# ShinobuAmasaki/forgex

Hardware: NVIDIA B200
Metric: input_GBps (higher is better)
Workload: dtype u8

## Files before the change

### forgex_b200/csrc/fx_cabi.cu

```cuda
#include <cuda_runtime.h>

#include <algorithm>
#include <atomic>
#include <cstdio>
#include <cstdlib>
#include <cstring>
#include <mutex>
#include <new>
#include <string>
#include <vector>

#include "../../include/forgex_b200.h"
#include "fx_internal.hpp"
#include "fx_kernels.cuh"

using namespace fxk;

namespace {

std::atomic<long long> g_launches{0};

constexpr int STATE_CAP = 16383;
constexpr int SPARSE_STATE_CAP = 2048;
constexpr int DIRECT_LIMIT_BYTES = 40 * 1024;
// ... 413 lines not shown
    if (n == 0) return FX_OK;
    if (p->prog.nfa_engine) return launch_nfa_bool(p, OP, buf, nullptr, stride, n, out, s);
    Plan pl;
    int rc = make_plan(p, pl);
    if (rc) return rc;
    int generic = gated_mode(p, OP);
    p->last_sparse = 0;
    p->last_compact = 0;
    if (OP == 1 && !generic && p->sparse && stride > 0 && n < (1ll << 31) && env_int("FX_SPARSE", 1)) {
        p->last_sparse = 1;
        return launch_sparse(p, pl, buf, nullptr, n, n * stride, out, s, stride);
    }
    if (pl.kind == 3 && p->compact && !generic && pl.kp.prefix_mode == 0 && stride >= 16 && stride % 16 == 0 &&
        reinterpret_cast<uintptr_t>(buf) % 16 == 0 && env_int("FX_COMPACT", 1)) {
        const bool in_smem = p->residency != FX_TABLE_GLOBAL;
        const size_t smem = 256 + (in_smem ? (size_t)p->prog.bt.nstates * 8 + 16 : 0);
        auto kern_s = k_bool_fixed_compact<OP, true>;
        auto kern_g = k_bool_fixed_compact<OP, false>;
        int bps = 0;
        int rc2 = in_smem ? occupancy_grid(kern_s, 1024, smem, p->dev.sm_count, bps) : occupancy_grid(kern_g, 1024, smem, p->dev.sm_count, bps);
        if (rc2) return rc2;
        long long want = (n + 1023) / 1024, cap = (long long)p->dev.sm_count * bps * 2;
        const int grid = (int)(want < cap ? want : cap);
        if (in_smem) kern_s<<<grid, 1024, smem, s>>>(pl.kp, p->dev.ctab4, p->dev.cmap4, buf, n, stride, out);
        else kern_g<<<grid, 1024, smem, s>>>(pl.kp, p->dev.ctab4, p->dev.cmap4, buf, n, stride, out);
        g_launches++;
        p->last_compact = in_smem ? 1 : 2;
        p->last_residency = in_smem ? FX_TABLE_SMEM : FX_TABLE_GLOBAL;
        return cuda_status(cudaGetLastError());
    }
    if (pl.kind == 0) return launch_fixed_v<OP, 0>(p, pl, buf, n, stride, out, s, generic);
    if (pl.kind == 2) return launch_fixed_v<OP, 2>(p, pl, buf, n, stride, out, s, generic);
    return launch_fixed_v<OP, 3>(p, pl, buf, n, stride, out, s, generic);
}

struct Tiling {
    int spt, cap;
    int64_t ntiles;
    int table_smem;
    size_t smem;
};

Tiling make_tiling(const Plan& pl, int64_t n, int64_t total, int extra = 0, int64_t max_cap = 1 << 30) {
    Tiling t;
    int64_t avg = n > 0 ? (total + n - 1) / n : 1;
    if (avg < 1) avg = 1;
    t.table_smem = (int)staged_bytes(pl);
    const int64_t per_cta = (227 * 1024) / 4 - 1024;
    int64_t spt = 0, cap = 0;
    for (int iter = 0; iter < 2; iter++) {
        int64_t fixed = tile_offset(t.table_smem, (int)(spt ? spt : 256)) + 64 + 128 + extra;
        cap = per_cta - fixed;
        if (cap < 8192) cap = 8192;
        if (cap > max_cap) cap = max_cap;
        cap &= ~(int64_t)127;
        spt = (cap * 4 / 5) / avg;
        spt = (spt / 32) * 32;
        if (spt < 32) spt = 32;
        if (spt > 2048) spt = 2048;
    }
    t.spt = (int)spt;
    t.cap = (int)cap;
    t.ntiles = (n + spt - 1) / spt;
    t.smem = (size_t)tile_offset(t.table_smem, t.spt) + (size_t)extra + (size_t)t.cap + 64;
    return t;
}

template <int OP, int KIND>
int launch_ragged_t(fx_pattern* p, const Plan& pl, const uint8_t* buf, const int64_t* off, int64_t n, int64_t total,
                    uint8_t* out, cudaStream_t s, int generic) {
    auto kern = k_bool_ragged<OP, KIND>;
    Tiling t = make_tiling(pl, n, total);
    int bps = 0;
    int rc = occupancy_grid(kern, 256, t.smem, p->dev.sm_count, bps);
    if (rc) return rc;
    long long cap = (long long)p->dev.sm_count * bps;
    int grid = (int)(t.ntiles < cap ? t.ntiles : cap);
    if (grid < 1) grid = 1;
    kern<<<grid, 256, t.smem, s>>>(pl.kp, buf, off, n, total, out, t.spt, t.cap, t.ntiles, t.table_smem, generic);
    g_launches++;
    return cuda_status(cudaGetLastError());
}

template <int KIND, int NR, bool HIGH, bool TWO>
int launch_sparse_t(fx_pattern* p, const Plan& pl, const SparseParams& sp, int table_bytes, const uint8_t* buf,
                    const int64_t* off, int64_t n, int64_t total, uint8_t* out, cudaStream_t s, int64_t stride) {
    auto kern = k_in_sparse<KIND, NR, HIGH, TWO>;
    int64_t avg = n > 0 ? (total + n - 1) / n : 1;
    if (avg < 1) avg = 1;
    int64_t want = (24 * 1024) / avg;
    const int spt = (int)(want < 32 ? 32 : want > 4096 ? 4096 : want);
    const int64_t ntiles = (n + spt - 1) / spt;
    const int table_smem = KIND == 3 ? 0 : (table_bytes + 15) & ~15;
    const size_t smem = (size_t)sparse_shared_head(table_smem) + 8 * (size_t)SPARSE_WARP_BYTES;
    int bps = 0;
    int rc = occupancy_grid(kern, 256, smem, p->dev.sm_count, bps);
    if (rc) return rc;
    long long cap = (long long)p->dev.sm_count * bps;
    long long wantg = (ntiles + 7) / 8;
    int grid = (int)(wantg < cap ? wantg : cap);
    if (grid < 1) grid = 1;
    const int prezeroed = sp.start_nul == 0 && pl.kp.q0_accepting == 0;
    if (prezeroed) CUDA_TRY(cudaMemsetAsync(out, 0, (size_t)n, s));
    kern<<<grid, 256, smem, s>>>(pl.kp, sp, buf, off, n, total, out, spt, ntiles, table_smem, prezeroed, stride);
    g_launches++;
    return cuda_status(cudaGetLastError());
}

template <int KIND, bool HIGH>
int launch_sparse_k(fx_pattern* p, const Plan& pl, const SparseParams& sp, int tb, const uint8_t* buf, const int64_t* off,
                    int64_t n, int64_t total, uint8_t* out, cudaStream_t s, int64_t stride) {
    if (p->first.sweep_nr == 1 && p->first.sweep_lo[0] == p->first.sweep_hi[0]) {
        const SparseParams& one = sp;
        if (p->first.two) return launch_sparse_t<KIND, -1, HIGH, true>(p, pl, one, tb, buf, off, n, total, out, s, stride);
        return launch_sparse_t<KIND, -1, HIGH, false>(p, pl, one, tb, buf, off, n, total, out, s, stride);
    }
    switch (p->first.sweep_nr) {
        case 0: return launch_sparse_t<KIND, 0, true, false>(p, pl, sp, tb, buf, off, n, total, out, s, stride);
        case 1: return launch_sparse_t<KIND, 1, HIGH, false>(p, pl, sp, tb, buf, off, n, total, out, s, stride);
        case 2: return launch_sparse_t<KIND, 2, HIGH, false>(p, pl, sp, tb, buf, off, n, total, out, s, stride);
        case 3: return launch_sparse_t<KIND, 3, HIGH, false>(p, pl, sp, tb, buf, off, n, total, out, s, stride);
        default: return launch_sparse_t<KIND, 4, HIGH, false>(p, pl, sp, tb, buf, off, n, total, out, s, stride);
    }
}

void fill_sweep(const FirstSet& f, SparseParams& sp) {
    for (int r = 0; r < 4; r++) {
        const int k = r < f.sweep_nr ? r : 0;
        sp.add_lo[r] = (0x80u - f.sweep_lo[k]) * 0x01010101u;
        sp.add_hi[r] = (0x7Fu - f.sweep_hi[k]) * 0x01010101u;
    }
    if (f.sweep_nr == 1 && f.sweep_lo[0] == f.sweep_hi[0]) sp.add_lo[0] = f.sweep_lo[0] * 0x01010101u;
    sp.second = f.second * 0x01010101u;
    sp.second_high = f.second_high ? 0xFFFFFFFFu : 0u;
}

int launch_sparse(fx_pattern* p, const Plan& pl, const uint8_t* buf, const int64_t* off, int64_t n, int64_t total,
                  uint8_t* out, cudaStream_t s, int64_t stride) {
    const fx::ByteTable& at = p->anchored.bt;
    const DeviceTables& d = p->dev;
    SparseParams sp;
    sp.table = d.a_table; sp.classmap = d.a_classmap; sp.flags = d.a_flags;
    sp.table_words = (int)at.table.size();
    sp.row_shift = at.row_shift;
    sp.q0 = at.q0; sp.start_nul = at.start_nul;
    fill_sweep(p->first, sp);
    const int tb = (int)at.table.size() * 2;
    const bool smem_table = p->residency != FX_TABLE_GLOBAL && tb <= 24 * 1024;
    if (smem_table)
        return p->first.high ? launch_sparse_k<2, true>(p, pl, sp, tb, buf, off, n, total, out, s, stride)
                             : launch_sparse_k<2, false>(p, pl, sp, tb, buf, off, n, total, out, s, stride);
    return p->first.high ? launch_sparse_k<3, true>(p, pl, sp, tb, buf, off, n, total, out, s, stride)
                         : launch_sparse_k<3, false>(p, pl, sp, tb, buf, off, n, total, out, s, stride);
}

template <int OP>
int launch_ragged(fx_pattern* p, const uint8_t* buf, const int64_t* off, int64_t n, int64_t total, uint8_t* out,
                  cudaStream_t s) {
    if (n < 0 || total < 0) return FX_ERR_BAD_ARGUMENT;
    if (n == 0) return FX_OK;
    if (p->prog.nfa_engine) return launch_nfa_bool(p, OP, buf, off, 0, n, out, s);
    Plan pl;
    int rc = make_plan(p, pl);
    if (rc) return rc;
    int generic = gated_mode(p, OP);
    p->last_sparse = 0;
    if (OP == 1 && !generic && p->sparse && n < (1ll << 31) && env_int("FX_SPARSE", 1)) {
        p->last_sparse = 1;
        return launch_sparse(p, pl, buf, off, n, total, out, s, 0);
    }
    if (pl.kind == 0) return launch_ragged_t<OP, 0>(p, pl, buf, off, n, total, out, s, generic);
    if (pl.kind == 2) return launch_ragged_t<OP, 2>(p, pl, buf, off, n, total, out, s, generic);
    return launch_ragged_t<OP, 3>(p, pl, buf, off, n, total, out, s, generic);
}

template <int KIND>
int launch_regex_ragged_t(fx_pattern* p, const Plan& pl, const uint8_t* buf, const int64_t* off, int64_t n,
                          int64_t total, int64_t* from, int64_t* to, cudaStream_t s) {
    auto kern = k_regex_ragged<KIND>;
    Tiling t = make_tiling(pl, n, total);
    int bps = 0;
    int rc = occupancy_grid(kern, 256, t.smem, p->dev.sm_count, bps);
    if (rc) return rc;
    long long cap = (long long)p->dev.sm_count * bps;
    int grid = (int)(t.ntiles < cap ? t.ntiles : cap);
    if (grid < 1) grid = 1;
    kern<<<grid, 256, t.smem, s>>>(pl.kp, buf, off, n, total, from, to, t.spt, t.cap, t.ntiles, t.table_smem);
    g_launches++;
    return cuda_status(cudaGetLastError());
// ... 1055 lines not shown
```

### forgex_b200/csrc/fx_kernels.cuh

```cuda
#pragma once
#include <cuda_runtime.h>
#include <stdint.h>

namespace fxk {

static constexpr uint32_t W_ACC = 0x8000u, W_INTER = 0x4000u, W_STATE = 0x3FFFu;
static constexpr uint32_t SF_ACC = 1, SF_END = 2, SF_INTER = 4, SF_MATCHED = 8, SF_FAILACC1 = 16;

struct KParams {
    const uint16_t* table;
    const uint8_t* classmap;
    const uint8_t* flags;
    const uint8_t* lits;
    int table_words;
    int nstates;
    int row_shift;
    int start, start_nul, q0, q0_accepting;
    int all_len, pre_len, suf_len;
    int all_active;
    int pre_active, suf_active;
    const uint16_t* a_table;
    const uint8_t* a_classmap;
    const uint8_t* a_flags;
    int a_row_shift, a_start_nul, a_q0;
// ... 706 lines not shown
    int64_t t1;
};
__device__ __forceinline__ TileCtx load_tile(const uint8_t* __restrict__ buf,
                                             const int64_t* __restrict__ offsets, int64_t n, int64_t total, int64_t t,
                                             int spt, int cap, uint8_t* tile, int32_t* s_off, uint32_t mbar,
                                             uint32_t& phase) {
    TileCtx c;
    c.first = t * spt;
    c.count = (int)((n - c.first) < spt ? (n - c.first) : spt);
    const int64_t t0 = __ldg(offsets + c.first);
    const int64_t tend = __ldg(offsets + c.first + c.count);
    c.t1 = tend - t0 > cap ? t0 + cap : tend;
    bool armed = false;
    c.base = t0;
    if (t0 < c.t1) c.base = stage_tile(buf, t0, c.t1, total, tile, mbar, armed);
    for (int i = threadIdx.x; i <= c.count; i += blockDim.x) {
        const int64_t o = __ldg(offsets + c.first + i);
        s_off[i] = o > c.t1 ? OFF_BEYOND : (int32_t)(o - c.base);
    }
    if (armed) { mbar_wait(mbar, phase); phase ^= 1; }
    __syncthreads();
    return c;
}

__host__ __device__ __forceinline__ int tile_offset(int table_smem_bytes, int spt) {
    return (16 + 256 + table_smem_bytes + (spt + 4) * 4 + spt + 127) & ~127;
}

template <int OP, int KIND>
__global__ void __launch_bounds__(256, 4) k_bool_ragged(KParams p, const uint8_t* __restrict__ buf,
                                                        const int64_t* __restrict__ offsets, int64_t n, int64_t total,
                                                        uint8_t* __restrict__ out, int spt, int cap, int64_t ntiles,
                                                        int table_smem_bytes, int generic) {
    extern __shared__ __align__(128) uint8_t smem[];
    uint8_t* s_cmap = smem + 16;
    uint8_t* s_table = smem + 16 + 256;
    int32_t* s_off = reinterpret_cast<int32_t*>(smem + 16 + 256 + table_smem_bytes);
    uint8_t* s_res = reinterpret_cast<uint8_t*>(s_off + spt + 4);
    uint8_t* tile = smem + tile_offset(table_smem_bytes, spt);
    const uint32_t mbar = smem_u32(smem);
    Table<KIND> T = stage_table<KIND>(p, s_table, s_cmap);
    if (threadIdx.x == 0) mbar_init(mbar, 1);
    __syncthreads();
    uint32_t phase = 0;
    const uint32_t tile_addr = smem_u32(tile);
    for (int64_t t = blockIdx.x; t < ntiles; t += gridDim.x) {
        const TileCtx c = load_tile(buf, offsets, n, total, t, spt, cap, tile, s_off, mbar, phase);
        for (int i = threadIdx.x; i < c.count; i += blockDim.x) {
            const int32_t r0 = s_off[i], r1 = s_off[i + 1];
            bool r;
            if (generic || r1 == OFF_BEYOND) {
                const int64_t o0 = __ldg(offsets + c.first + i), o1 = __ldg(offsets + c.first + i + 1);
                r = eval_bool_slow<OP>(p, buf + o0, o1 - o0);
            } else {
                const int len = r1 - r0;
                const uint32_t a = tile_addr + (uint32_t)r0;
                if (degenerate_text<OP>(len, len ? lds_u8(a) : 0)) r = p.q0_accepting != 0;
                else {
                    uint32_t high = 0;
                    r = result_flag(p, walk_smem(T, (uint32_t)p.start, a, len, high));
                    if (OP == 1 && r && p.prefix_mode == 1 && (high & 0x80808080u))
                        r = recheck_in_with_prefix(p, buf + (c.base + r0), len);
                }
            }
            s_res[i] = r ? 1 : 0;
        }
        __syncthreads();
        for (int i = threadIdx.x; i < c.count; i += blockDim.x) out[c.first + i] = s_res[i];
        __syncthreads();
    }
}

struct SparseParams {
    const uint16_t* table;
    const uint8_t* classmap;
    const uint8_t* flags;
    int table_words, row_shift, q0, start_nul;
    uint32_t add_lo[4];
    uint32_t add_hi[4];
    uint32_t second;
    uint32_t second_high;
};

static constexpr int SPARSE_WARP_BYTES = 2 * 64 * 16;
static constexpr int SPARSE_PARAM_BYTES = 1024;
__host__ __device__ __forceinline__ int sparse_shared_head(int table_smem_bytes) { return ((256 + table_smem_bytes + 15) & ~15) + SPARSE_PARAM_BYTES; }

template <int NR, bool HIGH>
__device__ __forceinline__ uint32_t first_mask(const SparseParams& sp, uint32_t w) {
    uint32_t m = 0;
    if (NR == -1) {
        const uint32_t x = w ^ sp.add_lo[0];
        m = (x - 0x01010101u) & ~x;
    } else {
        const uint32_t y = w & 0x7F7F7F7Fu;
#pragma unroll
        for (int r = 0; r < NR; r++) m |= (y + sp.add_lo[r]) & ~(y + sp.add_hi[r]);
    }
    if (HIGH) m |= w;
    return m;
}
__device__ __forceinline__ uint32_t lead_sel(const SparseParams& sp) { return sp.second_high ? 0xBA98u : 0x4444u; }
template <bool LEAD>
__device__ __forceinline__ uint32_t second_zero(const SparseParams& sp, uint32_t w, uint32_t sel) {
    uint32_t z = w ^ sp.second;
    if (LEAD) {
        uint32_t s;
        asm("prmt.b32 %0, %1, 0, %2;" : "=r"(s) : "r"(w), "r"(sel));
        z &= ~s;
    }
    return z;
}
__device__ __forceinline__ uint32_t pair_mask(const SparseParams& sp, uint32_t w, uint32_t z, uint32_t z_next) {
    const uint32_t t = (w ^ sp.add_lo[0]) | __funnelshift_r(z, z_next, 8);
    return (t - 0x01010101u) & ~t;
}
template <int NR, bool HIGH, bool TWO>
__device__ __forceinline__ uint32_t unit_any(const SparseParams& sp, const uint4& a, const uint4& b, uint32_t& seen,
                                             uint32_t z_next = 0u) {
    const uint32_t w[8] = {a.x, a.y, a.z, a.w, b.x, b.y, b.z, b.w};
    const uint32_t all = w[0] | w[1] | w[2] | w[3] | w[4] | w[5] | w[6] | w[7];
    seen |= all;
    uint32_t any = 0;
    if (TWO) {
        const uint32_t sel = lead_sel(sp);
#pragma unroll
        for (int k = 7; k >= 0; k--) {
            const uint32_t z = second_zero<!HIGH>(sp, w[k], sel);
            any |= pair_mask(sp, w[k], z, z_next);
            z_next = z;
        }
        if (HIGH) any |= all;
    } else {
#pragma unroll
        for (int k = 0; k < 8; k++) any |= first_mask<NR, false>(sp, w[k]);
        if (HIGH) any |= all;
    }
    return any & 0x80808080u;
}
__device__ __forceinline__ uint32_t pack_byte_flags(uint32_t m) { return ((((m >> 7) & 0x01010101u) * 0x00204081u) >> 21) & 0xFu; }

template <class TBL, class FETCH>
__device__ __forceinline__ bool attempt_wins(const Anchored& A, const TBL& T, FETCH fetch, int64_t len, uint32_t st, int64_t pos) {
    uint32_t w = st;
    int64_t seq = 0;
    bool inter = false;
    for (int64_t j = pos; j <= len; j++) {
        const uint32_t b = j < len ? fetch(j) : 0u;
        if (inter && (b & 0xC0) != 0x80) {
            const uint32_t f = __ldg(A.flags + (w & W_STATE));
            if (f & ((SF_FAILACC1 << (int)(j - seq)) - SF_FAILACC1)) return true;
            inter = false;
        }
        const uint32_t nw = T.next(w & W_STATE, b);
        if ((nw & W_INTER) && !inter) seq = j;
        inter = (nw & W_INTER) != 0;
        w = nw;
        if (w & W_ACC) return true;
        if ((w & W_STATE) == 0) return false;
    }
    return false;
}

struct SparseCtx {
    const uint8_t* buf;
    const int64_t* offsets;
    int64_t stride;
    uint8_t* out;
    int64_t n, total;
    int spt;
    uint4* units;
    uint4* starts;
};
static constexpr uint32_t SPARSE_START = 0, SPARSE_RECHECK = 2;
__device__ __forceinline__ int64_t sparse_off(const int64_t* __restrict__ offsets, int64_t stride, int64_t i) {
    return offsets ? __ldg(offsets + i) : i * stride;
}

template <int KIND>
__device__ __forceinline__ Table<KIND> sparse_table(const SparseParams& sp, uint32_t s_table, uint32_t s_cmap) {
    Table<KIND> T;
    T.s_table = s_table; T.s_cmap = s_cmap; T.g_table = sp.table; T.g_cmap = sp.classmap; T.shift = sp.row_shift;
    return T;
}

template <int KIND>
__device__ __noinline__ void sparse_run_starts(const KParams& p, const SparseParams& sp, uint32_t s_table, uint32_t s_cmap,
                                               const SparseCtx& c, int count) {
    const Table<KIND> T = sparse_table<KIND>(sp, s_table, s_cmap);
    const int lane = threadIdx.x & 31;
    const Anchored A{sp.flags, sp.start_nul, sp.q0};
    __syncwarp();
    if (lane < count) {
        const uint4 e = c.starts[lane];
        const int64_t first = (int64_t)e.x * c.spt;
        const int64_t* off = c.offsets + first;
        const uint32_t kind = e.y & 7u;
        const int64_t val = (int64_t)(((unsigned long long)e.w << 32) | e.z);
        if (c.offsets == nullptr) {
            const int64_t s = kind == SPARSE_START ? val / c.stride : val;
            const uint8_t* str = c.buf + (first + s) * c.stride;
            bool win;
            if (kind == SPARSE_START) {
                win = !(c.stride == 1 && __ldg(str) == 0x20) &&
                      attempt_wins(A, T, FetchGlobal{str}, c.stride, (uint32_t)sp.q0, val - s * c.stride);
                if (win && p.prefix_mode == 1 && (e.y >> 31)) win = recheck_in_with_prefix(p, str, c.stride);
                if (win) c.out[first + s] = 1;
            } else {
                c.out[first + s] = recheck_in_with_prefix(p, str, c.stride) ? 1 : 0;
            }
        } else if (kind == SPARSE_START) {
            const int cnt = (int)((c.n - first) < c.spt ? (c.n - first) : c.spt);
            int64_t vlo = __ldg(off), vhi = __ldg(off + cnt);
            const int64_t gpos = vlo + val;
            int s = 0, sh = cnt;
            for (int iter = 0; sh - s > 1; iter++) {
                int mid = (s + sh) >> 1;
                if (iter < 6) {
                    mid = s + (int)((float)(gpos - vlo) * (float)(sh - s) / (float)(vhi - vlo));
                    mid = mid <= s ? s + 1 : mid >= sh ? sh - 1 : mid;
                }
                const int64_t v = __ldg(off + mid);
                if (v <= gpos) { s = mid; vlo = v; } else { sh = mid; vhi = v; }
            }
            const int64_t o0 = __ldg(off + s), o1 = __ldg(off + s + 1);
            const uint8_t* str = c.buf + o0;
            if (!(o1 - o0 == 1 && __ldg(str) == 0x20)) {
                bool win = attempt_wins(A, T, FetchGlobal{str}, o1 - o0, (uint32_t)sp.q0, gpos - o0);
                if (win && p.prefix_mode == 1 && (e.y >> 31)) win = recheck_in_with_prefix(p, str, o1 - o0);
                if (win) c.out[first + s] = 1;
            }
        } else {
            const int64_t o0 = __ldg(off + val), o1 = __ldg(off + val + 1);
            c.out[first + val] = recheck_in_with_prefix(p, c.buf + o0, o1 - o0) ? 1 : 0;
        }
    }
    __syncwarp();
}

template <int KIND, int NR, bool HIGH, bool TWO>
__device__ __noinline__ int sparse_run_units(const KParams& p, const SparseParams& sp, uint32_t s_table, uint32_t s_cmap,
                                             const SparseCtx& c, int count, int sqn) {
    const Table<KIND> T = sparse_table<KIND>(sp, s_table, s_cmap);
    const int lane = threadIdx.x & 31;
    const uint32_t FULL = 0xffffffffu;
    __syncwarp();
    uint32_t cand = 0, tile = 0, flag = 0;
    int64_t P = 0, t0 = 0;
    if (lane < count) {
        const uint4 e = c.units[lane];
        tile = e.x; flag = e.y & 0x80000000u;
        const int64_t first = (int64_t)e.x * c.spt;
        const int cnt = (int)((c.n - first) < c.spt ? (c.n - first) : c.spt);
        t0 = sparse_off(c.offsets, c.stride, first);
        const int64_t tend = sparse_off(c.offsets, c.stride, first + cnt);
        const uintptr_t gbuf = reinterpret_cast<uintptr_t>(c.buf);
        const uintptr_t ua = ((gbuf + (uintptr_t)t0) & ~(uintptr_t)31) + ((((uintptr_t)e.w << 32) | e.z) << 5);
        const uint4 v0 = __ldg(reinterpret_cast<const uint4*>(ua)), v1 = __ldg(reinterpret_cast<const uint4*>(ua + 16));
        P = (int64_t)ua - (int64_t)gbuf;
        if (TWO) {
            const uint32_t sel = lead_sel(sp);
            uint32_t z_next = P + 32 < tend ? second_zero<true>(sp, __ldg(reinterpret_cast<const uint8_t*>(ua + 32)), sel) : 0u;
            const uint32_t w[8] = {v0.x, v0.y, v0.z, v0.w, v1.x, v1.y, v1.z, v1.w};
#pragma unroll
            for (int k = 7; k >= 0; k--) {
                const uint32_t z = second_zero<true>(sp, w[k], sel);
                cand |= pack_byte_flags(pair_mask(sp, w[k], z, z_next) | (HIGH ? w[k] : 0u)) << (4 * k);
                z_next = z;
            }
        } else {
            cand = pack_byte_flags(first_mask<NR, HIGH>(sp, v0.x)) | (pack_byte_flags(first_mask<NR, HIGH>(sp, v0.y)) << 4) |
                   (pack_byte_flags(first_mask<NR, HIGH>(sp, v0.z)) << 8) | (pack_byte_flags(first_mask<NR, HIGH>(sp, v0.w)) << 12) |
                   (pack_byte_flags(first_mask<NR, HIGH>(sp, v1.x)) << 16) | (pack_byte_flags(first_mask<NR, HIGH>(sp, v1.y)) << 20) |
                   (pack_byte_flags(first_mask<NR, HIGH>(sp, v1.z)) << 24) | (pack_byte_flags(first_mask<NR, HIGH>(sp, v1.w)) << 28);
        }
        if (P < t0) cand &= 0xFFFFFFFFu << (int)(t0 - P);
        if (P + 32 > tend) cand &= (P >= tend) ? 0u : (0xFFFFFFFFu >> (int)(P + 32 - tend));
    }
    while (__any_sync(FULL, cand != 0)) {
        bool sv = false;
        int64_t pos = 0;
        if (cand) {
            pos = P + __ffs(cand) - 1;
            cand &= cand - 1;
            const uint32_t b = __ldg(c.buf + pos);
            const uint32_t w1 = T.next((uint32_t)sp.q0, b);
            if (w1 & (W_ACC | W_INTER)) sv = true;
            else if (w1 & W_STATE) {
                const uint32_t b1 = pos + 1 < c.total ? __ldg(c.buf + pos + 1) : 0u;
                sv = ((T.next(w1, b1) | T.next(w1, 0u)) & (W_STATE | W_ACC)) != 0;
            }
        }
        const uint32_t m = __ballot_sync(FULL, sv);
        if (m) {
            const unsigned long long rel = (unsigned long long)(pos - t0);
            if (sv) c.starts[sqn + __popc(m & ((1u << lane) - 1))] = make_uint4(tile, SPARSE_START | flag, (uint32_t)rel, (uint32_t)(rel >> 32));
            sqn += __popc(m);
            if (sqn >= 32) {
                sparse_run_starts<KIND>(p, sp, s_table, s_cmap, c, 32);
                if (lane < sqn - 32) { const uint4 x = c.starts[32 + lane]; c.starts[lane] = x; }
                sqn -= 32;
                __syncwarp();
            }
        }
    }
    __syncwarp();
    return sqn;
}

static constexpr int SPARSE_CTAS_PER_SM = 4, SPARSE_ROWS = 4;

template <int NR, bool HIGH, bool TWO, bool WHOLE>
__device__ __forceinline__ uint32_t sweep_group(const SparseParams& sp, uintptr_t sbase, int r, int lim, uint32_t& seen) {
    const int lane = threadIdx.x & 31;
    uint4 va[SPARSE_ROWS], vb[SPARSE_ROWS];
#pragma unroll
    for (int k = 0; k < SPARSE_ROWS; k++) {
        const int u = ((r + k) << 5) + lane;
        const uintptr_t a = sbase + ((uintptr_t)(uint32_t)u << 5);
        if (WHOLE || u < lim) {
            va[k] = ldg_nc_v4(reinterpret_cast<const void*>(a));
            vb[k] = ldg_nc_v4(reinterpret_cast<const void*>(a + 16));
        } else {
            va[k] = make_uint4(0, 0, 0, 0); vb[k] = va[k];
        }
    }
    uint32_t zn[SPARSE_ROWS];
    if (TWO) {
        const uint32_t sel = lead_sel(sp);
        uint32_t z0[SPARSE_ROWS];
#pragma unroll
        for (int k = 0; k < SPARSE_ROWS; k++) z0[k] = second_zero<true>(sp, va[k].x, sel);
#pragma unroll
        for (int k = 0; k < SPARSE_ROWS; k++) {
            const uint32_t give = lane != 0 ? z0[k] : k + 1 < SPARSE_ROWS ? z0[k + 1] : 0u;
            zn[k] = __shfl_sync(0xffffffffu, give, (lane + 1) & 31);
            if (!WHOLE && ((r + k) << 5) + lane + 1 >= lim) zn[k] = 0u;
        }
    }
    uint32_t bits = 0;
#pragma unroll
    for (int k = 0; k < SPARSE_ROWS; k++) {
        const int u = ((r + k) << 5) + lane;
        const uint32_t h = (WHOLE || u < lim) ? unit_any<NR, HIGH, TWO>(sp, va[k], vb[k], seen, TWO ? zn[k] : 0u) : 0u;
        bits |= (h ? 1u : 0u) << k;
    }
    return bits;
}

template <int KIND, int NR, bool HIGH, bool TWO>
__global__ void __launch_bounds__(256, SPARSE_CTAS_PER_SM) k_in_sparse(KParams p, SparseParams sp, const uint8_t* __restrict__ buf,
                                                                     const int64_t* __restrict__ offsets, int64_t n, int64_t total,
                                                                     uint8_t* __restrict__ out, int spt, int64_t ntiles,
                                                                     int table_smem_bytes, int prezeroed, int64_t stride) {
    extern __shared__ __align__(128) uint8_t smem[];
    uint8_t* s_cmap = smem;
    uint8_t* s_table = smem + 256;
    const int warp = threadIdx.x >> 5, lane = threadIdx.x & 31;
    uint4* s_units = reinterpret_cast<uint4*>(smem + sparse_shared_head(table_smem_bytes) + warp * SPARSE_WARP_BYTES);
    uint4* s_starts = s_units + 64;
    KParams anch = p;
    anch.table = sp.table; anch.classmap = sp.classmap; anch.table_words = sp.table_words; anch.row_shift = sp.row_shift;
    Table<KIND> T = stage_table<KIND>(anch, s_table, s_cmap);
    static_assert(sizeof(KParams) + sizeof(SparseParams) + 8 * sizeof(SparseCtx) <= SPARSE_PARAM_BYTES, "parameter block");
    uint8_t* s_params = smem + sparse_shared_head(table_smem_bytes) - SPARSE_PARAM_BYTES;
    KParams* sh_p = reinterpret_cast<KParams*>(s_params);
    SparseParams* sh_sp = reinterpret_cast<SparseParams*>(s_params + sizeof(KParams));
    SparseCtx* sh_c = reinterpret_cast<SparseCtx*>(s_params + sizeof(KParams) + sizeof(SparseParams)) + warp;
    if (threadIdx.x == 0) { *sh_p = p; *sh_sp = sp; }
    if (lane == 0) {
        sh_c->buf = buf; sh_c->offsets = offsets; sh_c->stride = stride; sh_c->out = out; sh_c->n = n; sh_c->total = total;
        sh_c->spt = spt;
        sh_c->units = s_units; sh_c->starts = s_starts;
    }
    __syncthreads();
    const Anchored A{sp.flags, sp.start_nul, sp.q0};
    const uint32_t FULL = 0xffffffffu;
    const int nt = (int)ntiles;

    enum { ST_NEW = 0, ST_SWEEP = 1, ST_STRINGS = 2, ST_PUSH = 3 };
    int t = blockIdx.x * 8 + warp;
    int st = ST_NEW, it = 0;
    int uqn = 0, sqn = 0;
    int count = 0, nrows = 0;
    int64_t seg = 0, nunits = 0;
    uintptr_t ubase = 0;
    uint32_t hitbits = 0;
    bool high = false;
    int64_t nx0 = 0, nx1 = 0;
    bool have_next = false;

    bool drain = false;
    for (;;) {
        for (;;) {
            if (uqn >= 32 || sqn >= 32 || drain) break;
            if (st == ST_NEW) {
                if (t >= nt) { drain = true; break; }
                const int64_t first = (int64_t)t * spt;
                count = (int)((n - first) < spt ? (n - first) : spt);
                const int64_t t0 = have_next ? nx0 : sparse_off(offsets, stride, first);
                const int64_t tend = have_next ? nx1 : sparse_off(offsets, stride, first + count);
                {
                    const int64_t fn = first + (int64_t)gridDim.x * 8 * spt;
                    have_next = fn < n;
                    if (have_next) { nx0 = sparse_off(offsets, stride, fn); nx1 = sparse_off(offsets, stride, fn + spt < n ? fn + spt : n); }
                }
                const uintptr_t g0 = reinterpret_cast<uintptr_t>(buf) + (uintptr_t)t0;
                ubase = g0 & ~(uintptr_t)31;
                nunits = tend > t0 ? (int64_t)((reinterpret_cast<uintptr_t>(buf) + (uintptr_t)tend - ubase + 31) >> 5) : 0;
                seg = 0;
                high = nunits > 1024;
                st = ST_SWEEP;
            }
            if (st == ST_SWEEP) {
                const int64_t left = nunits - seg;
                const int lim = (int)(left < 1024 ? left : 1024);
                const uintptr_t sbase = ubase + ((uintptr_t)seg << 5);
                nrows = (lim + 31) >> 5;
                hitbits = 0;
                uint32_t seen = 0;
                int r = 0;
                for (; ((r + SPARSE_ROWS) << 5) <= lim; r += SPARSE_ROWS)
                    hitbits |= sweep_group<NR, HIGH, TWO, true>(sp, sbase, r, lim, seen) << r;
                if (r < nrows) hitbits |= sweep_group<NR, HIGH, TWO, false>(sp, sbase, r, lim, seen) << r;
                high = high || __any_sync(FULL, (seen & 0x80808080u) != 0);
                st = seg == 0 ? ST_STRINGS : ST_PUSH;
                it = 0;
            }
            if (st == ST_STRINGS) {
                const int64_t first = (int64_t)t * spt;
                if (prezeroed) it = count;
                while (it < count && sqn < 32) {
                    const int i = it + lane;
                    bool r = false, defer = false;
                    if (i < count) {
                        const int64_t o0 = sparse_off(offsets, stride, first + i), o1 = sparse_off(offsets, stride, first + i + 1);
                        const int64_t len = o1 - o0;
                        if (len == 0 || (len == 1 && __ldg(buf + o0) == 0x20)) r = p.q0_accepting != 0;
                        else if (sp.start_nul != 0) {
                            r = attempt_wins(A, T, FetchGlobal{buf + o0}, len, (uint32_t)sp.start_nul, 0);
                            if (r && p.prefix_mode == 1 && high) { r = false; defer = true; }
                        }
                        out[first + i] = r ? 1 : 0;
                    }
                    const uint32_t m = __ballot_sync(FULL, defer);
                    if (defer) s_starts[sqn + __popc(m & ((1u << lane) - 1))] = make_uint4((uint32_t)t, SPARSE_RECHECK, (uint32_t)i, 0u);
                    sqn += __popc(m);
                    it += 32;
                }
                if (it < count) continue;
                __syncwarp();
                st = ST_PUSH;
                it = 0;
            }
            while (it < nrows && uqn < 32) {
                const bool hit = (hitbits >> it) & 1u;
                const uint32_t m = __ballot_sync(FULL, hit);
                if (hit) {
                    const unsigned long long u = (unsigned long long)(seg + ((int64_t)it << 5) + lane);
                    s_units[uqn + __popc(m & ((1u << lane) - 1))] = make_uint4((uint32_t)t, high ? 0x80000000u : 0u, (uint32_t)u, (uint32_t)(u >> 32));
                }
                uqn += __popc(m);
                it++;
            }
            if (it < nrows) continue;
            seg += (int64_t)nrows << 5;
            if (seg < nunits) st = ST_SWEEP;
            else {
                st = ST_NEW;
                t += gridDim.x * 8;
            }
        }
        if (uqn >= 32 || (drain && uqn > 0)) {
            const int run = uqn < 32 ? uqn : 32;
            sqn = sparse_run_units<KIND, NR, HIGH, TWO>(*sh_p, *sh_sp, T.s_table, T.s_cmap, *sh_c, run, sqn);
            if (lane < uqn - run) { const uint4 x = s_units[run + lane]; s_units[lane] = x; }
            uqn -= run;
            __syncwarp();
        } else if (sqn >= 32 || (drain && sqn > 0)) {
            const int run = sqn < 32 ? sqn : 32;
            sparse_run_starts<KIND>(*sh_p, *sh_sp, T.s_table, T.s_cmap, *sh_c, run);
            if (lane < sqn - run) { const uint4 x = s_starts[run + lane]; s_starts[lane] = x; }
            sqn -= run;
            __syncwarp();
        } else {
            drain = false;
            if (st == ST_NEW && t >= nt) break;
        }
    }
}

template <int KIND>
__global__ void __launch_bounds__(256) k_regex_ragged(KParams p, const uint8_t* __restrict__ buf,
                                                      const int64_t* __restrict__ offsets, int64_t n, int64_t total,
                                                      int64_t* __restrict__ from, int64_t* __restrict__ to,
                                                      int spt, int cap, int64_t ntiles, int table_smem_bytes) {
    extern __shared__ __align__(128) uint8_t smem[];
    uint8_t* s_cmap = smem + 16;
    uint8_t* s_table = smem + 16 + 256;
    int32_t* s_off = reinterpret_cast<int32_t*>(smem + 16 + 256 + table_smem_bytes);
    uint8_t* tile = smem + tile_offset(table_smem_bytes, spt);
    const uint32_t mbar = smem_u32(smem);
    Table<KIND> T = stage_table<KIND>(p, s_table, s_cmap);
    if (threadIdx.x == 0) mbar_init(mbar, 1);
    __syncthreads();
    uint32_t phase = 0;
    const uint32_t tile_addr = smem_u32(tile);
    const bool plain = !p.all_active && !p.pre_active;
    for (int64_t t = blockIdx.x; t < ntiles; t += gridDim.x) {
        const TileCtx c = load_tile(buf, offsets, n, total, t, spt, cap, tile, s_off, mbar, phase);
        for (int i = threadIdx.x; i < c.count; i += blockDim.x) {
            const int32_t r0 = s_off[i], r1 = s_off[i + 1];
            int64_t f, e;
            if (r1 == OFF_BEYOND) {
                const int64_t o0 = __ldg(offsets + c.first + i), o1 = __ldg(offsets + c.first + i + 1);
                eval_regex(p, T, FetchGlobal{buf + o0}, o1 - o0, f, e);
            } else if (plain) {
                const int len = r1 - r0;
                const uint32_t a = tile_addr + (uint32_t)r0;
                f = 0; e = 0;
                if (!(len == 0 || (len == 1 && lds_u8(a) == 0x20))) {
                    int64_t ff, tt;
                    brute_force_smem(Anchored{p.flags, p.start_nul, p.q0}, T, a, len, ff, tt);
                    if (ff > 0 && tt > 0) { f = ff; e = tt; }
                }
            } else {
                eval_regex(p, T, FetchShared{tile_addr + (uint32_t)r0}, (int64_t)(r1 - r0), f, e);
            }
            from[c.first + i] = f;
            to[c.first + i] = e;
        }
        __syncthreads();
    }
}

static constexpr uint32_t W_SSTATE = 0x0FFFu, W_RA = 0x3000u;
static constexpr int SPAN_ROW = 258;
struct SpanParams {
    const uint16_t* direct;
    const uint16_t* table;
    const uint8_t* classmap;
    const uint8_t* endinfo;
    int nstates, row_shift, start, start_acc;
    const uint16_t* rdelta;
    const uint8_t* rpage;
    const uint8_t* rmixed;
    const int32_t* cuts;
    int rstates, rclasses, rstart, nul_class, ffff_class, nmixed;
};

template <int FK>
struct SpanFwd {
    uint32_t s_table, s_cmap;
    const uint16_t* g_table;
    const uint8_t* g_cmap;
    int shift;
    __device__ __forceinline__ uint32_t next(uint32_t st, uint32_t b) const {
        if (FK == 0) return lds_u16(s_table + st * (SPAN_ROW * 2) + b * 2);
        if (FK == 1) return lds_u16(s_table + (((st << shift) + lds_u8(s_cmap + b)) << 1));
        return __ldg(g_table + ((st << shift) + __ldg(g_cmap + b)));
    }
};
template <bool RS>
struct SpanRev {
    uint32_t s_delta, s_page, s_mixed;
    __device__ __forceinline__ uint32_t delta(const SpanParams& sp, uint32_t r, uint32_t c) const {
        if (RS) return lds_u16(s_delta + ((r * (uint32_t)sp.rclasses + c) << 1));
        return __ldg(sp.rdelta + r * (uint32_t)sp.rclasses + c);
    }
    __device__ __forceinline__ uint32_t cls(const SpanParams& sp, uint32_t cp) const {
// ... 1450 lines not shown
```

Baseline: 4104.

## Restructure sparse IN kernel into sweep-to-bitmap then per-chunk candidate verification

Result: faster. 4411 (median of 6 runs) (+7.5%).

```diff
diff --git a/forgex_b200/csrc/fx_cabi.cu b/forgex_b200/csrc/fx_cabi.cu
--- a/forgex_b200/csrc/fx_cabi.cu
+++ b/forgex_b200/csrc/fx_cabi.cu
@@ -519,6 +519,28 @@
     return cuda_status(cudaGetLastError());
 }
 
+int scratch_pool(int dev, cudaMemPool_t& pool) {
+    static std::mutex mu;
+    static std::vector<cudaMemPool_t> pools;
+    std::lock_guard<std::mutex> lock(mu);
+    if (dev < 0) return FX_ERR_BAD_ARGUMENT;
+    if ((size_t)dev >= pools.size()) pools.resize((size_t)dev + 1, nullptr);
+    if (!pools[(size_t)dev]) {
+        cudaMemPoolProps props;
+        memset(&props, 0, sizeof(props));
+        props.allocType = cudaMemAllocationTypePinned;
+        props.location.type = cudaMemLocationTypeDevice;
+        props.location.id = dev;
+        cudaMemPool_t mp = nullptr;
+        CUDA_TRY(cudaMemPoolCreate(&mp, &props));
+        uint64_t keep = 1ull << 30;
+        CUDA_TRY(cudaMemPoolSetAttribute(mp, cudaMemPoolAttrReleaseThreshold, &keep));
+        pools[(size_t)dev] = mp;
+    }
+    pool = pools[(size_t)dev];
+    return FX_OK;
+}
+
 template <int KIND, int NR, bool HIGH, bool TWO>
 int launch_sparse_t(fx_pattern* p, const Plan& pl, const SparseParams& sp, int table_bytes, const uint8_t* buf,
                     const int64_t* off, int64_t n, int64_t total, uint8_t* out, cudaStream_t s, int64_t stride) {
@@ -537,11 +559,20 @@
     long long wantg = (ntiles + 7) / 8;
     int grid = (int)(wantg < cap ? wantg : cap);
     if (grid < 1) grid = 1;
-    const int prezeroed = sp.start_nul == 0 && pl.kp.q0_accepting == 0;
-    if (prezeroed) CUDA_TRY(cudaMemsetAsync(out, 0, (size_t)n, s));
-    kern<<<grid, 256, smem, s>>>(pl.kp, sp, buf, off, n, total, out, spt, ntiles, table_smem, prezeroed, stride);
+    const uintptr_t g = reinterpret_cast<uintptr_t>(buf);
+    const int64_t units = (int64_t)(((g + (uintptr_t)total + 31) >> 5) - (g >> 5));
+    const size_t bitmap_bytes = ((size_t)sparse_tile_words(units, ntiles) + 1) * 4;
+    cudaMemPool_t pool = nullptr;
+    rc = scratch_pool(p->dev.device, pool);
+    if (rc) return rc;
+    void* scratch = nullptr;
+    CUDA_TRY(cudaMallocFromPoolAsync(&scratch, bitmap_bytes, pool, s));
+    uint32_t* hits = static_cast<uint32_t*>(scratch);
+    kern<<<grid, 256, smem, s>>>(pl.kp, sp, buf, off, n, total, out, spt, ntiles, table_smem, stride, hits);
     g_launches++;
-    return cuda_status(cudaGetLastError());
+    const cudaError_t e = cudaGetLastError();
+    const cudaError_t f = cudaFreeAsync(scratch, s);
+    return cuda_status(e != cudaSuccess ? e : f);
 }
 
 template <int KIND, bool HIGH>
diff --git a/forgex_b200/csrc/fx_kernels.cuh b/forgex_b200/csrc/fx_kernels.cuh
--- a/forgex_b200/csrc/fx_kernels.cuh
+++ b/forgex_b200/csrc/fx_kernels.cuh
@@ -812,10 +812,6 @@
     uint32_t second_high;
 };
 
-static constexpr int SPARSE_WARP_BYTES = 2 * 64 * 16;
-static constexpr int SPARSE_PARAM_BYTES = 1024;
-__host__ __device__ __forceinline__ int sparse_shared_head(int table_smem_bytes) { return ((256 + table_smem_bytes + 15) & ~15) + SPARSE_PARAM_BYTES; }
-
 template <int NR, bool HIGH>
 __device__ __forceinline__ uint32_t first_mask(const SparseParams& sp, uint32_t w) {
     uint32_t m = 0;
@@ -892,151 +888,11 @@
     return false;
 }
 
-struct SparseCtx {
-    const uint8_t* buf;
-    const int64_t* offsets;
-    int64_t stride;
-    uint8_t* out;
-    int64_t n, total;
-    int spt;
-    uint4* units;
-    uint4* starts;
-};
-static constexpr uint32_t SPARSE_START = 0, SPARSE_RECHECK = 2;
 __device__ __forceinline__ int64_t sparse_off(const int64_t* __restrict__ offsets, int64_t stride, int64_t i) {
     return offsets ? __ldg(offsets + i) : i * stride;
 }
 
-template <int KIND>
-__device__ __forceinline__ Table<KIND> sparse_table(const SparseParams& sp, uint32_t s_table, uint32_t s_cmap) {
-    Table<KIND> T;
-    T.s_table = s_table; T.s_cmap = s_cmap; T.g_table = sp.table; T.g_cmap = sp.classmap; T.shift = sp.row_shift;
-    return T;
-}
-
-template <int KIND>
-__device__ __noinline__ void sparse_run_starts(const KParams& p, const SparseParams& sp, uint32_t s_table, uint32_t s_cmap,
-                                               const SparseCtx& c, int count) {
-    const Table<KIND> T = sparse_table<KIND>(sp, s_table, s_cmap);
-    const int lane = threadIdx.x & 31;
-    const Anchored A{sp.flags, sp.start_nul, sp.q0};
-    __syncwarp();
-    if (lane < count) {
-        const uint4 e = c.starts[lane];
-        const int64_t first = (int64_t)e.x * c.spt;
-        const int64_t* off = c.offsets + first;
-        const uint32_t kind = e.y & 7u;
-        const int64_t val = (int64_t)(((unsigned long long)e.w << 32) | e.z);
-        if (c.offsets == nullptr) {
-            const int64_t s = kind == SPARSE_START ? val / c.stride : val;
-            const uint8_t* str = c.buf + (first + s) * c.stride;
-            bool win;
-            if (kind == SPARSE_START) {
-                win = !(c.stride == 1 && __ldg(str) == 0x20) &&
-                      attempt_wins(A, T, FetchGlobal{str}, c.stride, (uint32_t)sp.q0, val - s * c.stride);
-                if (win && p.prefix_mode == 1 && (e.y >> 31)) win = recheck_in_with_prefix(p, str, c.stride);
-                if (win) c.out[first + s] = 1;
-            } else {
-                c.out[first + s] = recheck_in_with_prefix(p, str, c.stride) ? 1 : 0;
-            }
-        } else if (kind == SPARSE_START) {
-            const int cnt = (int)((c.n - first) < c.spt ? (c.n - first) : c.spt);
-            int64_t vlo = __ldg(off), vhi = __ldg(off + cnt);
-            const int64_t gpos = vlo + val;
-            int s = 0, sh = cnt;
-            for (int iter = 0; sh - s > 1; iter++) {
-                int mid = (s + sh) >> 1;
-                if (iter < 6) {
-                    mid = s + (int)((float)(gpos - vlo) * (float)(sh - s) / (float)(vhi - vlo));
-                    mid = mid <= s ? s + 1 : mid >= sh ? sh - 1 : mid;
-                }
-                const int64_t v = __ldg(off + mid);
-                if (v <= gpos) { s = mid; vlo = v; } else { sh = mid; vhi = v; }
-            }
-            const int64_t o0 = __ldg(off + s), o1 = __ldg(off + s + 1);
-            const uint8_t* str = c.buf + o0;
-            if (!(o1 - o0 == 1 && __ldg(str) == 0x20)) {
-                bool win = attempt_wins(A, T, FetchGlobal{str}, o1 - o0, (uint32_t)sp.q0, gpos - o0);
-                if (win && p.prefix_mode == 1 && (e.y >> 31)) win = recheck_in_with_prefix(p, str, o1 - o0);
-                if (win) c.out[first + s] = 1;
-            }
-        } else {
-            const int64_t o0 = __ldg(off + val), o1 = __ldg(off + val + 1);
-            c.out[first + val] = recheck_in_with_prefix(p, c.buf + o0, o1 - o0) ? 1 : 0;
-        }
-    }
-    __syncwarp();
-}
-
-template <int KIND, int NR, bool HIGH, bool TWO>
-__device__ __noinline__ int sparse_run_units(const KParams& p, const SparseParams& sp, uint32_t s_table, uint32_t s_cmap,
-                                             const SparseCtx& c, int count, int sqn) {
-    const Table<KIND> T = sparse_table<KIND>(sp, s_table, s_cmap);
-    const int lane = threadIdx.x & 31;
-    const uint32_t FULL = 0xffffffffu;
-    __syncwarp();
-    uint32_t cand = 0, tile = 0, flag = 0;
-    int64_t P = 0, t0 = 0;
-    if (lane < count) {
-        const uint4 e = c.units[lane];
-        tile = e.x; flag = e.y & 0x80000000u;
-        const int64_t first = (int64_t)e.x * c.spt;
-        const int cnt = (int)((c.n - first) < c.spt ? (c.n - first) : c.spt);
-        t0 = sparse_off(c.offsets, c.stride, first);
-        const int64_t tend = sparse_off(c.offsets, c.stride, first + cnt);
-        const uintptr_t gbuf = reinterpret_cast<uintptr_t>(c.buf);
-        const uintptr_t ua = ((gbuf + (uintptr_t)t0) & ~(uintptr_t)31) + ((((uintptr_t)e.w << 32) | e.z) << 5);
-        const uint4 v0 = __ldg(reinterpret_cast<const uint4*>(ua)), v1 = __ldg(reinterpret_cast<const uint4*>(ua + 16));
-        P = (int64_t)ua - (int64_t)gbuf;
-        if (TWO) {
-            const uint32_t sel = lead_sel(sp);
-            uint32_t z_next = P + 32 < tend ? second_zero<true>(sp, __ldg(reinterpret_cast<const uint8_t*>(ua + 32)), sel) : 0u;
-            const uint32_t w[8] = {v0.x, v0.y, v0.z, v0.w, v1.x, v1.y, v1.z, v1.w};
-#pragma unroll
-            for (int k = 7; k >= 0; k--) {
-                const uint32_t z = second_zero<true>(sp, w[k], sel);
-                cand |= pack_byte_flags(pair_mask(sp, w[k], z, z_next) | (HIGH ? w[k] : 0u)) << (4 * k);
-                z_next = z;
-            }
-        } else {
-            cand = pack_byte_flags(first_mask<NR, HIGH>(sp, v0.x)) | (pack_byte_flags(first_mask<NR, HIGH>(sp, v0.y)) << 4) |
-                   (pack_byte_flags(first_mask<NR, HIGH>(sp, v0.z)) << 8) | (pack_byte_flags(first_mask<NR, HIGH>(sp, v0.w)) << 12) |
-                   (pack_byte_flags(first_mask<NR, HIGH>(sp, v1.x)) << 16) | (pack_byte_flags(first_mask<NR, HIGH>(sp, v1.y)) << 20) |
-                   (pack_byte_flags(first_mask<NR, HIGH>(sp, v1.z)) << 24) | (pack_byte_flags(first_mask<NR, HIGH>(sp, v1.w)) << 28);
-        }
-        if (P < t0) cand &= 0xFFFFFFFFu << (int)(t0 - P);
-        if (P + 32 > tend) cand &= (P >= tend) ? 0u : (0xFFFFFFFFu >> (int)(P + 32 - tend));
-    }
-    while (__any_sync(FULL, cand != 0)) {
-        bool sv = false;
-        int64_t pos = 0;
-        if (cand) {
-            pos = P + __ffs(cand) - 1;
-            cand &= cand - 1;
-            const uint32_t b = __ldg(c.buf + pos);
-            const uint32_t w1 = T.next((uint32_t)sp.q0, b);
-            if (w1 & (W_ACC | W_INTER)) sv = true;
-            else if (w1 & W_STATE) {
-                const uint32_t b1 = pos + 1 < c.total ? __ldg(c.buf + pos + 1) : 0u;
-                sv = ((T.next(w1, b1) | T.next(w1, 0u)) & (W_STATE | W_ACC)) != 0;
-            }
-        }
-        const uint32_t m = __ballot_sync(FULL, sv);
-        if (m) {
-            const unsigned long long rel = (unsigned long long)(pos - t0);
-            if (sv) c.starts[sqn + __popc(m & ((1u << lane) - 1))] = make_uint4(tile, SPARSE_START | flag, (uint32_t)rel, (uint32_t)(rel >> 32));
-            sqn += __popc(m);
-            if (sqn >= 32) {
-                sparse_run_starts<KIND>(p, sp, s_table, s_cmap, c, 32);
-                if (lane < sqn - 32) { const uint4 x = c.starts[32 + lane]; c.starts[lane] = x; }
-                sqn -= 32;
-                __syncwarp();
-            }
-        }
-    }
-    __syncwarp();
-    return sqn;
-}
+__host__ __device__ __forceinline__ int64_t sparse_tile_words(int64_t u0, int64_t t) { return (u0 >> 5) + t; }
 
 static constexpr int SPARSE_CTAS_PER_SM = 4, SPARSE_ROWS = 4;
 
@@ -1078,144 +934,185 @@
     return bits;
 }
 
+template <int NR, bool HIGH, bool TWO>
+__device__ __forceinline__ bool sparse_sweep_tile(const SparseParams& sp, uintptr_t ubase, int64_t nunits, uint32_t* words) {
+    const int lane = threadIdx.x & 31;
+    const uint32_t FULL = 0xffffffffu;
+    bool high = nunits > 1024;
+    for (int64_t seg = 0; seg < nunits; seg += 1024) {
+        const int64_t left = nunits - seg;
+        const int lim = (int)(left < 1024 ? left : 1024);
+        const int nrows = (lim + 31) >> 5;
+        const uintptr_t sbase = ubase + ((uintptr_t)seg << 5);
+        uint32_t hitbits = 0, seen = 0;
+        int r = 0;
+        for (; ((r + SPARSE_ROWS) << 5) <= lim; r += SPARSE_ROWS)
+            hitbits |= sweep_group<NR, HIGH, TWO, true>(sp, sbase, r, lim, seen) << r;
+        if (r < nrows) hitbits |= sweep_group<NR, HIGH, TWO, false>(sp, sbase, r, lim, seen) << r;
+        high = high || __any_sync(FULL, (seen & 0x80808080u) != 0);
+        uint32_t mine = 0;
+        for (int k = 0; k < nrows; k++) {
+            const uint32_t b = __ballot_sync(FULL, (hitbits >> k) & 1u);
+            if (lane == k) mine = b;
+        }
+        if (lane < nrows) words[(seg >> 5) + lane] = mine;
+    }
+    return high;
+}
+
+static constexpr int SPARSE_CHUNK = 256;
+static constexpr int SPARSE_WARP_BYTES = (SPARSE_CHUNK + 1) * 8 + SPARSE_CHUNK + 32 * 4;
+__host__ __device__ __forceinline__ int sparse_shared_head(int table_smem_bytes) { return (256 + table_smem_bytes + 15) & ~15; }
+
 template <int KIND, int NR, bool HIGH, bool TWO>
 __global__ void __launch_bounds__(256, SPARSE_CTAS_PER_SM) k_in_sparse(KParams p, SparseParams sp, const uint8_t* __restrict__ buf,
                                                                      const int64_t* __restrict__ offsets, int64_t n, int64_t total,
                                                                      uint8_t* __restrict__ out, int spt, int64_t ntiles,
-                                                                     int table_smem_bytes, int prezeroed, int64_t stride) {
+                                                                     int table_smem_bytes, int64_t stride, uint32_t* hits) {
     extern __shared__ __align__(128) uint8_t smem[];
     uint8_t* s_cmap = smem;
     uint8_t* s_table = smem + 256;
     const int warp = threadIdx.x >> 5, lane = threadIdx.x & 31;
-    uint4* s_units = reinterpret_cast<uint4*>(smem + sparse_shared_head(table_smem_bytes) + warp * SPARSE_WARP_BYTES);
-    uint4* s_starts = s_units + 64;
+    uint8_t* wsm = smem + sparse_shared_head(table_smem_bytes) + warp * SPARSE_WARP_BYTES;
+    int64_t* s_off = reinterpret_cast<int64_t*>(wsm);
+    uint8_t* s_res = wsm + (SPARSE_CHUNK + 1) * 8;
+    uint32_t* s_list = reinterpret_cast<uint32_t*>(s_res + SPARSE_CHUNK);
     KParams anch = p;
     anch.table = sp.table; anch.classmap = sp.classmap; anch.table_words = sp.table_words; anch.row_shift = sp.row_shift;
-    Table<KIND> T = stage_table<KIND>(anch, s_table, s_cmap);
-    static_assert(sizeof(KParams) + sizeof(SparseParams) + 8 * sizeof(SparseCtx) <= SPARSE_PARAM_BYTES, "parameter block");
-    uint8_t* s_params = smem + sparse_shared_head(table_smem_bytes) - SPARSE_PARAM_BYTES;
-    KParams* sh_p = reinterpret_cast<KParams*>(s_params);
-    SparseParams* sh_sp = reinterpret_cast<SparseParams*>(s_params + sizeof(KParams));
-    SparseCtx* sh_c = reinterpret_cast<SparseCtx*>(s_params + sizeof(KParams) + sizeof(SparseParams)) + warp;
-    if (threadIdx.x == 0) { *sh_p = p; *sh_sp = sp; }
-    if (lane == 0) {
-        sh_c->buf = buf; sh_c->offsets = offsets; sh_c->stride = stride; sh_c->out = out; sh_c->n = n; sh_c->total = total;
-        sh_c->spt = spt;
-        sh_c->units = s_units; sh_c->starts = s_starts;
-    }
+    const Table<KIND> T = stage_table<KIND>(anch, s_table, s_cmap);
     __syncthreads();
+    const int nt = (int)ntiles;
     const Anchored A{sp.flags, sp.start_nul, sp.q0};
     const uint32_t FULL = 0xffffffffu;
-    const int nt = (int)ntiles;
-
-    enum { ST_NEW = 0, ST_SWEEP = 1, ST_STRINGS = 2, ST_PUSH = 3 };
-    int t = blockIdx.x * 8 + warp;
-    int st = ST_NEW, it = 0;
-    int uqn = 0, sqn = 0;
-    int count = 0, nrows = 0;
-    int64_t seg = 0, nunits = 0;
-    uintptr_t ubase = 0;
-    uint32_t hitbits = 0;
-    bool high = false;
+    const uintptr_t gbuf = reinterpret_cast<uintptr_t>(buf), gbase = gbuf & ~(uintptr_t)31;
+    const bool per_string = p.q0_accepting != 0 || sp.start_nul != 0;
     int64_t nx0 = 0, nx1 = 0;
     bool have_next = false;
-
-    bool drain = false;
-    for (;;) {
-        for (;;) {
-            if (uqn >= 32 || sqn >= 32 || drain) break;
-            if (st == ST_NEW) {
-                if (t >= nt) { drain = true; break; }
-                const int64_t first = (int64_t)t * spt;
-                count = (int)((n - first) < spt ? (n - first) : spt);
-                const int64_t t0 = have_next ? nx0 : sparse_off(offsets, stride, first);
-                const int64_t tend = have_next ? nx1 : sparse_off(offsets, stride, first + count);
-                {
-                    const int64_t fn = first + (int64_t)gridDim.x * 8 * spt;
-                    have_next = fn < n;
-                    if (have_next) { nx0 = sparse_off(offsets, stride, fn); nx1 = sparse_off(offsets, stride, fn + spt < n ? fn + spt : n); }
+    for (int t = blockIdx.x * 8 + warp; t < nt; t += gridDim.x * 8) {
+        const int64_t first = (int64_t)t * spt;
+        const int cnt = (int)((n - first) < spt ? (n - first) : spt);
+        const int64_t t0 = have_next ? nx0 : sparse_off(offsets, stride, first);
+        const int64_t tend = have_next ? nx1 : sparse_off(offsets, stride, first + cnt);
+        {
+            const int64_t fn = first + (int64_t)gridDim.x * 8 * spt;
+            have_next = fn < n;
+            if (have_next) { nx0 = sparse_off(offsets, stride, fn); nx1 = sparse_off(offsets, stride, fn + spt < n ? fn + spt : n); }
+        }
+        const uintptr_t ubase = (gbuf + (uintptr_t)t0) & ~(uintptr_t)31;
+        const int64_t nunits = tend > t0 ? (int64_t)((gbuf + (uintptr_t)tend - ubase + 31) >> 5) : 0;
+        uint32_t* words = hits + sparse_tile_words((int64_t)((ubase - gbase) >> 5), t);
+        const bool high = sparse_sweep_tile<NR, HIGH, TWO>(sp, ubase, nunits, words);
+        __syncwarp();
+        for (int c0 = 0; c0 < cnt; c0 += SPARSE_CHUNK) {
+            const int cc = cnt - c0 < SPARSE_CHUNK ? cnt - c0 : SPARSE_CHUNK;
+            const int64_t cf = first + c0;
+            if (offsets) {
+                int64_t o[SPARSE_CHUNK / 32 + 1];
+#pragma unroll
+                for (int k = 0; k <= SPARSE_CHUNK / 32; k++) o[k] = lane + 32 * k <= cc ? __ldg(offsets + cf + lane + 32 * k) : 0;
+#pragma unroll
+                for (int k = 0; k <= SPARSE_CHUNK / 32; k++) if (lane + 32 * k <= cc) s_off[lane + 32 * k] = o[k];
+            } else {
+                for (int i = lane; i <= cc; i += 32) s_off[i] = (cf + i) * stride;
+            }
+            __syncwarp();
+            const int64_t lo = s_off[0], hi = s_off[cc];
+            for (int i = lane; i < cc; i += 32) {
+                bool r = false;
+                if (per_string) {
+                    const int64_t o0 = s_off[i], len = s_off[i + 1] - o0;
+                    if (len == 0 || (len == 1 && __ldg(buf + o0) == 0x20)) r = p.q0_accepting != 0;
+                    else if (sp.start_nul != 0) {
+                        r = attempt_wins(A, T, FetchGlobal{buf + o0}, len, (uint32_t)sp.start_nul, 0);
+                        if (r && p.prefix_mode == 1 && high) r = recheck_in_with_prefix(p, buf + o0, len);
+                    }
                 }
-                const uintptr_t g0 = reinterpret_cast<uintptr_t>(buf) + (uintptr_t)t0;
-                ubase = g0 & ~(uintptr_t)31;
-                nunits = tend > t0 ? (int64_t)((reinterpret_cast<uintptr_t>(buf) + (uintptr_t)tend - ubase + 31) >> 5) : 0;
-                seg = 0;
-                high = nunits > 1024;
-                st = ST_SWEEP;
-            }
-            if (st == ST_SWEEP) {
-                const int64_t left = nunits - seg;
-                const int lim = (int)(left < 1024 ? left : 1024);
-                const uintptr_t sbase = ubase + ((uintptr_t)seg << 5);
-                nrows = (lim + 31) >> 5;
-                hitbits = 0;
-                uint32_t seen = 0;
-                int r = 0;
-                for (; ((r + SPARSE_ROWS) << 5) <= lim; r += SPARSE_ROWS)
-                    hitbits |= sweep_group<NR, HIGH, TWO, true>(sp, sbase, r, lim, seen) << r;
-                if (r < nrows) hitbits |= sweep_group<NR, HIGH, TWO, false>(sp, sbase, r, lim, seen) << r;
-                high = high || __any_sync(FULL, (seen & 0x80808080u) != 0);
-                st = seg == 0 ? ST_STRINGS : ST_PUSH;
-                it = 0;
-            }
-            if (st == ST_STRINGS) {
-                const int64_t first = (int64_t)t * spt;
-                if (prezeroed) it = count;
-                while (it < count && sqn < 32) {
-                    const int i = it + lane;
-                    bool r = false, defer = false;
-                    if (i < count) {
-                        const int64_t o0 = sparse_off(offsets, stride, first + i), o1 = sparse_off(offsets, stride, first + i + 1);
-                        const int64_t len = o1 - o0;
-                        if (len == 0 || (len == 1 && __ldg(buf + o0) == 0x20)) r = p.q0_accepting != 0;
-                        else if (sp.start_nul != 0) {
-                            r = attempt_wins(A, T, FetchGlobal{buf + o0}, len, (uint32_t)sp.start_nul, 0);
-                            if (r && p.prefix_mode == 1 && high) { r = false; defer = true; }
+                s_res[i] = r ? 1 : 0;
+            }
+            __syncwarp();
+            const int64_t ua = hi > lo ? (int64_t)(((gbuf + (uintptr_t)lo) & ~(uintptr_t)31) - ubase) >> 5 : 0;
+            const int64_t ub = hi > lo ? (int64_t)((gbuf + (uintptr_t)hi + 31 - ubase) >> 5) : 0;
+            for (int64_t w0 = ua >> 5; (w0 << 5) < ub; w0 += 32) {
+                const int64_t wi = w0 + lane;
+                uint32_t word = (wi << 5) < ub ? words[wi] : 0u;
+                const int64_t u = wi << 5;
+                if (u < ua) word = ua - u >= 32 ? 0u : word & (0xFFFFFFFFu << (int)(ua - u));
+                if (u + 32 > ub) word = u >= ub ? 0u : word & (0xFFFFFFFFu >> (int)(u + 32 - ub));
+                const int mine = __popc(word);
+                int before = mine;
+#pragma unroll
+                for (int d = 1; d < 32; d <<= 1) { const int x = __shfl_up_sync(FULL, before, d); if (lane >= d) before += x; }
+                const int all = __shfl_sync(FULL, before, 31);
+                before -= mine;
+                for (int b0 = 0; b0 < all; b0 += 32) {
+                    while (word && before < b0 + 32) {
+                        s_list[before - b0] = (uint32_t)(((wi - w0) << 5) + __ffs(word) - 1);
+                        word &= word - 1;
+                        before++;
+                    }
+                    __syncwarp();
+                    uint32_t cand = 0;
+                    int64_t P = 0;
+                    if (lane < all - b0) {
+                        const uintptr_t ua_addr = ubase + ((uintptr_t)(w0 << 5) + s_list[lane]) * 32;
+                        const uint4 v0 = __ldg(reinterpret_cast<const uint4*>(ua_addr)), v1 = __ldg(reinterpret_cast<const uint4*>(ua_addr + 16));
+                        P = (int64_t)(ua_addr - gbuf);
+                        if (TWO) {
+                            const uint32_t sel = lead_sel(sp);
+                            uint32_t z_next = P + 32 < tend ? second_zero<true>(sp, __ldg(reinterpret_cast<const uint8_t*>(ua_addr + 32)), sel) : 0u;
+                            const uint32_t w[8] = {v0.x, v0.y, v0.z, v0.w, v1.x, v1.y, v1.z, v1.w};
+#pragma unroll
+                            for (int k = 7; k >= 0; k--) {
+                                const uint32_t z = second_zero<true>(sp, w[k], sel);
+                                cand |= pack_byte_flags(pair_mask(sp, w[k], z, z_next) | (HIGH ? w[k] : 0u)) << (4 * k);
+                                z_next = z;
+                            }
+                        } else {
+                            const uint32_t w[8] = {v0.x, v0.y, v0.z, v0.w, v1.x, v1.y, v1.z, v1.w};
+#pragma unroll
+                            for (int k = 0; k < 8; k++) cand |= pack_byte_flags(first_mask<NR, HIGH>(sp, w[k])) << (4 * k);
                         }
-                        out[first + i] = r ? 1 : 0;
+                        if (P < lo) cand &= 0xFFFFFFFFu << (int)(lo - P);
+                        if (P + 32 > hi) cand &= (P >= hi) ? 0u : (0xFFFFFFFFu >> (int)(P + 32 - hi));
                     }
-                    const uint32_t m = __ballot_sync(FULL, defer);
-                    if (defer) s_starts[sqn + __popc(m & ((1u << lane) - 1))] = make_uint4((uint32_t)t, SPARSE_RECHECK, (uint32_t)i, 0u);
-                    sqn += __popc(m);
-                    it += 32;
+                    __syncwarp();
+                    while (cand) {
+                        const int64_t pos = P + __ffs(cand) - 1;
+                        cand &= cand - 1;
+                        const uint32_t b = __ldg(buf + pos);
+                        bool sv;
+                        if (TWO && b < 0x80) sv = true;
+                        else {
+                            const uint32_t w1 = T.next((uint32_t)sp.q0, b);
+                            sv = (w1 & (W_ACC | W_INTER)) != 0;
+                            if (!sv && (w1 & W_STATE)) {
+                                const uint32_t b1 = pos + 1 < total ? __ldg(buf + pos + 1) : 0u;
+                                sv = ((T.next(w1, b1) | T.next(w1, 0u)) & (W_STATE | W_ACC)) != 0;
+                            }
+                        }
+                        if (!sv) continue;
+                        int s;
+                        if (offsets) {
+                            int sh = cc;
+                            s = 0;
+                            while (sh - s > 1) {
+                                const int mid = (s + sh) >> 1;
+                                if (s_off[mid] <= pos) s = mid; else sh = mid;
+                            }
+                        } else {
+                            s = (int)(pos / stride - cf);
+                        }
+                        const int64_t o0 = s_off[s], len = s_off[s + 1] - o0;
+                        if (len == 1 && __ldg(buf + o0) == 0x20) continue;
+                        bool win = attempt_wins(A, T, FetchGlobal{buf + o0}, len, (uint32_t)sp.q0, pos - o0);
+                        if (win && p.prefix_mode == 1 && high) win = recheck_in_with_prefix(p, buf + o0, len);
+                        if (win) s_res[s] = 1;
+                    }
                 }
-                if (it < count) continue;
-                __syncwarp();
-                st = ST_PUSH;
-                it = 0;
-            }
-            while (it < nrows && uqn < 32) {
-                const bool hit = (hitbits >> it) & 1u;
-                const uint32_t m = __ballot_sync(FULL, hit);
-                if (hit) {
-                    const unsigned long long u = (unsigned long long)(seg + ((int64_t)it << 5) + lane);
-                    s_units[uqn + __popc(m & ((1u << lane) - 1))] = make_uint4((uint32_t)t, high ? 0x80000000u : 0u, (uint32_t)u, (uint32_t)(u >> 32));
-                }
-                uqn += __popc(m);
-                it++;
-            }
-            if (it < nrows) continue;
-            seg += (int64_t)nrows << 5;
-            if (seg < nunits) st = ST_SWEEP;
-            else {
-                st = ST_NEW;
-                t += gridDim.x * 8;
-            }
-        }
-        if (uqn >= 32 || (drain && uqn > 0)) {
-            const int run = uqn < 32 ? uqn : 32;
-            sqn = sparse_run_units<KIND, NR, HIGH, TWO>(*sh_p, *sh_sp, T.s_table, T.s_cmap, *sh_c, run, sqn);
-            if (lane < uqn - run) { const uint4 x = s_units[run + lane]; s_units[lane] = x; }
-            uqn -= run;
+            }
             __syncwarp();
-        } else if (sqn >= 32 || (drain && sqn > 0)) {
-            const int run = sqn < 32 ? sqn : 32;
-            sparse_run_starts<KIND>(*sh_p, *sh_sp, T.s_table, T.s_cmap, *sh_c, run);
-            if (lane < sqn - run) { const uint4 x = s_starts[run + lane]; s_starts[lane] = x; }
-            sqn -= run;
+            for (int i = lane; i < cc; i += 32) out[cf + i] = s_res[i];
             __syncwarp();
-        } else {
-            drain = false;
-            if (st == ST_NEW && t >= nt) break;
         }
     }
 }
```
